# AntreasAntoniou/HowToTrainYourMAMLPytorch

Measured on AMD Instinct MI355X. Metric: meta-tasks/sec, higher is better.
Workload: dtype bf16; 1 GPU; model=maml++_miniimagenet_5w1s, global_batch=128, tasks_per_gpu=128, ways=5, shots=1, targets=15, filters=48, inner_steps=5, msl=True, parallelism=task-dp1

## Files before the change

### howtotrainyourmamlpytorch_amd/ops/hip/bindings.cpp

```cpp
#include <torch/extension.h>
#include <vector>

std::vector<torch::Tensor> bn_act_fwd(torch::Tensor x, torch::Tensor gamma,
                                      torch::Tensor beta, double eps,
                                      double slope, bool act);
std::vector<torch::Tensor> bn_act_bwd(torch::Tensor dy, torch::Tensor x,
                                      torch::Tensor mean, torch::Tensor rstd,
                                      torch::Tensor gamma, torch::Tensor beta,
                                      double slope, bool act);
std::vector<torch::Tensor> bn_act_pool_fwd(torch::Tensor x, torch::Tensor gamma,
                                           torch::Tensor beta, double eps,
                                           double slope,
                                           c10::optional<torch::Tensor> sums_in);
std::vector<torch::Tensor> bn_act_pool_bwd(torch::Tensor dyp, torch::Tensor mask,
                                           torch::Tensor x, torch::Tensor mean,
                                           torch::Tensor rstd, torch::Tensor gamma,
                                           torch::Tensor beta, double slope);
std::vector<torch::Tensor> maxpool2x2_fwd(torch::Tensor x);
torch::Tensor maxpool2x2_bwd(torch::Tensor dy, torch::Tensor mask, long H, long W);
std::vector<torch::Tensor> ce_fwd(torch::Tensor logits, torch::Tensor labels);
torch::Tensor ce_bwd(torch::Tensor probs, torch::Tensor labels, torch::Tensor gtask);
std::vector<torch::Tensor> ce_dbwd(torch::Tensor probs, torch::Tensor labels,
                                   torch::Tensor gdl, torch::Tensor gtask);
std::vector<torch::Tensor> bn_act_dbwd(torch::Tensor x, torch::Tensor u,
                                       torch::Tensor gx, torch::Tensor mean,
                                       torch::Tensor rstd, torch::Tensor gamma,
                                       torch::Tensor beta, torch::Tensor ggam,
                                       torch::Tensor gbet, double slope, bool act);
std::vector<torch::Tensor> ln_act_fwd(torch::Tensor x, torch::Tensor bias,
                                      double eps, double slope, bool act);
std::vector<torch::Tensor> ln_act_bwd(torch::Tensor dy, torch::Tensor x,
                                      torch::Tensor mean, torch::Tensor rstd,
                                      torch::Tensor bias, double slope, bool act);
std::vector<torch::Tensor> ln_act_dbwd(torch::Tensor x, torch::Tensor dy,
                                       torch::Tensor gx, torch::Tensor gb,
                                       torch::Tensor mean, torch::Tensor rstd,
                                       torch::Tensor bias, double slope, bool act);
torch::Tensor lslr_fwd(torch::Tensor arena, torch::Tensor grad, torch::Tensor lr_vec);
std::vector<torch::Tensor> lslr_bwd(torch::Tensor gout, torch::Tensor grad,
                                    torch::Tensor lr_vec);
torch::Tensor tconv_repack(torch::Tensor w, bool dgrad);
std::vector<torch::Tensor> tconv_mm(torch::Tensor x, torch::Tensor wp,
                                    c10::optional<torch::Tensor> bias, long pad,
// ... 37 lines not shown
torch::Tensor gavgpool_bwd(torch::Tensor dy, long H, long W);
void adam_step(std::vector<torch::Tensor> params,
               std::vector<torch::Tensor> grads,
               std::vector<torch::Tensor> exp_avgs,
               std::vector<torch::Tensor> exp_avg_sqs,
               long step, double lr, double beta1, double beta2, double eps,
               double weight_decay, double clamp_v);

PYBIND11_MODULE(TORCH_EXTENSION_NAME, m) {
  m.def("bn_act_fwd", &bn_act_fwd, "fused task-batched BN+leakyReLU fwd");
  m.def("bn_act_bwd", &bn_act_bwd, "fused task-batched BN+leakyReLU bwd");
  m.def("bn_act_pool_fwd", &bn_act_pool_fwd, "fused BN+leakyReLU+maxpool fwd");
  m.def("bn_act_pool_bwd", &bn_act_pool_bwd, "fused BN+leakyReLU+maxpool bwd");
  m.def("maxpool2x2_fwd", &maxpool2x2_fwd, "NHWC maxpool 2x2 fwd");
  m.def("maxpool2x2_bwd", &maxpool2x2_bwd, "NHWC maxpool 2x2 bwd");
  m.def("ce_fwd", &ce_fwd, "fused softmax-CE fwd");
  m.def("ce_dbwd", &ce_dbwd, "softmax-CE double-backward");
  m.def("bn_act_dbwd", &bn_act_dbwd, "BN+leakyReLU analytic double-backward");
  m.def("ce_bwd", &ce_bwd, "fused softmax-CE bwd");
  m.def("ln_act_fwd", &ln_act_fwd, "fused task-batched LayerNorm+bias+leakyReLU fwd");
  m.def("ln_act_bwd", &ln_act_bwd, "fused task-batched LayerNorm+bias+leakyReLU bwd");
  m.def("ln_act_dbwd", &ln_act_dbwd, "LayerNorm+bias+leakyReLU analytic double-backward");
  m.def("lslr_fwd", &lslr_fwd, "fused LSLR arena update fwd");
  m.def("lslr_bwd", &lslr_bwd, "fused LSLR arena update bwd");
  m.def("tconv_repack", &tconv_repack, "repack conv weights for MFMA (fwd/dgrad)");
  m.def("tconv_mm", &tconv_mm, "task-batched MFMA 3x3 conv fwd/dgrad");
  m.def("tconv_wgrad", &tconv_wgrad, "task-batched MFMA 3x3 conv wgrad");
  m.def("tconv_repack_v2", &tconv_repack_v2,
        "repack conv weights into the v2 swizzled LDS image");
  m.def("tconv_mm_v2", &tconv_mm_v2,
        "async-pipelined MFMA 3x3 conv fwd/dgrad (v2)");
  m.def("tconv_wgrad_v2", &tconv_wgrad_v2,
        "async-pipelined wgrad via k-contiguous operand transposes (v2)");
// ... 24 lines not shown
```

### howtotrainyourmamlpytorch_amd/ops/hip/bn_act.hip

```cpp

#include "common.h"

using namespace maml355;

template <typename scalar_t>
__global__ void bn_sums_vec_kernel(const scalar_t* __restrict__ x,
                                   float* __restrict__ partials,
                                   int T, long M, int C, int rows_per_block) {
  const int c8n = C / 8;
  const int rows_in_block = blockDim.x / c8n;
  const int c8 = threadIdx.x % c8n;
  const int rg = threadIdx.x / c8n;
  const int t = blockIdx.x;
  const long row0 = (long)blockIdx.y * rows_per_block;
  extern __shared__ float ls[];
  float s[8] = {0}, q[8] = {0};
  if (rg < rows_in_block) {
    const scalar_t* xt = x + (long)t * M * C + c8 * 8;
    const long row_end = min(row0 + rows_per_block, M);
    for (long m = row0 + rg; m < row_end; m += rows_in_block) {
      float v[8];
      load8(xt + m * C, v);
#pragma unroll
      for (int j = 0; j < 8; ++j) { s[j] += v[j]; q[j] += v[j] * v[j]; }
// ... 17 lines not shown
      }
    }
    __syncthreads();
    n_ = step;
  }
  if (rg == 0) {
    float* pt = partials + (((long)t * gridDim.y + blockIdx.y) * 2) * C;
#pragma unroll
    for (int j = 0; j < 8; ++j) {
      pt[c8 * 8 + j] = ls[0 * C + c8 * 8 + j];
      pt[C + c8 * 8 + j] = ls[1 * C + c8 * 8 + j];
    }
  }
}

__global__ void bn_reduce2_kernel(const float* __restrict__ partials,
                                  float* __restrict__ sums, int T, int nblk,
                                  int C) {
  const int i = blockIdx.x * blockDim.x + threadIdx.x;
  if (i >= T * C) return;
  const int t = i / C, c = i % C;
  float s = 0.f, q = 0.f;
  for (int b = 0; b < nblk; ++b) {
    const float* p = partials + (((long)t * nblk + b) * 2) * C;
    s += p[c];
    q += p[C + c];
  }
  sums[((long)t * 2 + 0) * C + c] = s;
  sums[((long)t * 2 + 1) * C + c] = q;
}

template <typename scalar_t, bool PER_TASK_AFFINE, bool ACT>
__global__ void bn_norm_act_vec_kernel(const scalar_t* __restrict__ x,
                                       scalar_t* __restrict__ y,
                                       const float* __restrict__ mean,
                                       const float* __restrict__ rstd,
                                       const float* __restrict__ gamma,
                                       const float* __restrict__ beta,
                                       int T, long M, int C, float slope,
                                       int rows_per_block) {
  const int c8n = C / 8;
  const int rows_in_block = blockDim.x / c8n;
  const int c8 = threadIdx.x % c8n;
  const int rg = threadIdx.x / c8n;
// ... 515 lines not shown
    }
    const float s1 = bsums[((long)t * 2 + 0) * C + c];
    const float s2 = bsums[((long)t * 2 + 1) * C + c];
    dx[i] = from_f32<scalar_t>(g * rs * (d - s1 * invM - xh * s2 * invM));
  }
}

#include <torch/extension.h>
#include <ATen/cuda/CUDAContext.h>

namespace {

constexpr int kRowsPerBlock = 256;
constexpr int kThreads = 256;

template <typename scalar_t>
void bn_fwd_impl(const torch::Tensor& x, const torch::Tensor& gamma,
                 const torch::Tensor& beta, torch::Tensor& y,
                 torch::Tensor& sums, torch::Tensor& mean, torch::Tensor& var,
                 torch::Tensor& rstd, double eps, double slope, bool act,
                 int T, long M, int C) {
  auto stream = at::cuda::getCurrentCUDAStream();
  const bool per_task = gamma.dim() == 2;
  const bool vec = (C % 8 == 0) && C <= 512;
  const int cpad = ((C + WAVE - 1) / WAVE) * WAVE;
  dim3 sums_grid(T, (unsigned)((M + kRowsPerBlock - 1) / kRowsPerBlock));
  const int threads = cpad * std::max<int>(1, kThreads / cpad);
  const int lds_bytes = 2 * threads * sizeof(float);
  if (vec) {
    const int rpb = 1024;
    const int nb = (int)((M + rpb - 1) / rpb);
    dim3 g(T, (unsigned)nb);
    auto partials = torch::empty({T, nb, 2, C},
                                 x.options().dtype(torch::kFloat32));
    hipLaunchKernelGGL((bn_sums_vec_kernel<scalar_t>), g, dim3(256),
                       16384, stream.stream(),
                       reinterpret_cast<const scalar_t*>(x.data_ptr()),
                       partials.data_ptr<float>(), T, M, C, rpb);
    hipLaunchKernelGGL(bn_reduce2_kernel, dim3((T * C + 255) / 256), dim3(256),
                       0, stream.stream(), partials.data_ptr<float>(),
                       sums.data_ptr<float>(), T, nb, C);
  } else
  hipLaunchKernelGGL((bn_sums_kernel<scalar_t>), sums_grid, dim3(threads),
                     lds_bytes, stream.stream(),
                     reinterpret_cast<const scalar_t*>(x.data_ptr()), sums.data_ptr<float>(), T, M, C,
                     kRowsPerBlock);
  const int fin_threads = 256;
  const int fin_blocks = (T * C + fin_threads - 1) / fin_threads;
  hipLaunchKernelGGL(bn_finalize_kernel, dim3(fin_blocks), dim3(fin_threads), 0,
                     stream.stream(), sums.data_ptr<float>(),
                     mean.data_ptr<float>(), var.data_ptr<float>(),
                     rstd.data_ptr<float>(), T, M, C, (float)eps);
  const long total = (long)T * M * C;
#define LAUNCH_NORM(PT, ACT_)                                                  \
  do {                                                                         \
    if (vec) {                                                                 \
// ... 12 lines not shown
                         reinterpret_cast<scalar_t*>(y.data_ptr()),            \
                         mean.data_ptr<float>(), rstd.data_ptr<float>(),       \
                         gamma.data_ptr<float>(), beta.data_ptr<float>(),      \
                         T, M, C, (float)slope);                               \
    }                                                                          \
  } while (0)
  if (per_task) { if (act) LAUNCH_NORM(true, true); else LAUNCH_NORM(true, false); }
  else { if (act) LAUNCH_NORM(false, true); else LAUNCH_NORM(false, false); }
#undef LAUNCH_NORM
}

template <typename scalar_t>
void bn_bwd_impl(const torch::Tensor& dy, const torch::Tensor& x,
                 const torch::Tensor& mean, const torch::Tensor& rstd,
                 const torch::Tensor& gamma, const torch::Tensor& beta,
                 torch::Tensor& bsums, torch::Tensor& dx, double slope,
                 bool act, int T, long M, int C) {
  auto stream = at::cuda::getCurrentCUDAStream();
  const bool per_task = gamma.dim() == 2;
  const bool vec = (C % 8 == 0) && C <= 512;
  const int cpad = ((C + WAVE - 1) / WAVE) * WAVE;
  dim3 sums_grid(T, (unsigned)((M + kRowsPerBlock - 1) / kRowsPerBlock));
  const int threads = cpad * std::max<int>(1, kThreads / cpad);
  const int lds_bytes = 2 * threads * sizeof(float);
  const long total = (long)T * M * C;
#define LAUNCH_BWD(PT, ACT_)                                                   \
  do {                                                                         \
    if (vec) {                                                                 \
      const int nb = (int)((M + 1023) / 1024);                                 \
      dim3 gs(T, (unsigned)nb);                                                \
      auto partials = torch::empty({T, nb, 2, C},                              \
                                   x.options().dtype(torch::kFloat32));        \
      hipLaunchKernelGGL((bn_bwd_sums_vec_kernel<scalar_t, PT, ACT_>),         \
                         gs, dim3(256), 16384,                                 \
                         stream.stream(),                                      \
                         reinterpret_cast<const scalar_t*>(dy.data_ptr()),     \
                         reinterpret_cast<const scalar_t*>(x.data_ptr()),      \
                         mean.data_ptr<float>(), rstd.data_ptr<float>(),       \
                         gamma.data_ptr<float>(), beta.data_ptr<float>(),      \
                         partials.data_ptr<float>(), T, M, C, (float)slope,    \
                         1024);                                                \
      hipLaunchKernelGGL(bn_reduce2_kernel, dim3((T * C + 255) / 256),         \
                         dim3(256), 0, stream.stream(),                        \
                         partials.data_ptr<float>(),                           \
                         bsums.data_ptr<float>(), T, nb, C);                   \
      hipLaunchKernelGGL((bn_bwd_dx_vec_kernel<scalar_t, PT, ACT_>),           \
                         sums_grid, dim3(256), 0, stream.stream(),             \
                         reinterpret_cast<const scalar_t*>(dy.data_ptr()),     \
                         reinterpret_cast<const scalar_t*>(x.data_ptr()),      \
                         reinterpret_cast<scalar_t*>(dx.data_ptr()),           \
                         mean.data_ptr<float>(), rstd.data_ptr<float>(),       \
                         gamma.data_ptr<float>(), beta.data_ptr<float>(),      \
                         bsums.data_ptr<float>(), T, M, C, (float)slope,       \
                         kRowsPerBlock);                                       \
      break;                                                                   \
    }                                                                          \
    hipLaunchKernelGGL((bn_bwd_sums_kernel<scalar_t, PT, ACT_>), sums_grid,    \
                       dim3(threads), lds_bytes, stream.stream(),              \
                       reinterpret_cast<const scalar_t*>(dy.data_ptr()),       \
                       reinterpret_cast<const scalar_t*>(x.data_ptr()),        \
// ... 14 lines not shown
  if (per_task) { if (act) LAUNCH_BWD(true, true); else LAUNCH_BWD(true, false); }
  else { if (act) LAUNCH_BWD(false, true); else LAUNCH_BWD(false, false); }
#undef LAUNCH_BWD
}

}

std::vector<torch::Tensor> bn_act_fwd(torch::Tensor x, torch::Tensor gamma,
                                      torch::Tensor beta, double eps,
                                      double slope, bool act) {
  TORCH_CHECK(x.is_cuda() && x.dim() == 3 && x.is_contiguous());
  const int T = (int)x.size(0);
  const long M = x.size(1);
  const int C = (int)x.size(2);
  auto opts = x.options().dtype(torch::kFloat32);
  auto sums = torch::zeros({T, 2, C}, opts);
  auto mean = torch::empty({T, C}, opts);
  auto var = torch::empty({T, C}, opts);
  auto rstd = torch::empty({T, C}, opts);
  auto y = torch::empty_like(x);
  auto gc = gamma.contiguous().to(torch::kFloat32);
  auto bc = beta.contiguous().to(torch::kFloat32);
  if (x.scalar_type() == torch::kFloat32) {
    bn_fwd_impl<float>(x, gc, bc, y, sums, mean, var, rstd, eps, slope, act, T, M, C);
  } else if (x.scalar_type() == torch::kBFloat16) {
    bn_fwd_impl<__hip_bfloat16>(x, gc, bc, y, sums, mean, var, rstd, eps, slope, act, T, M, C);
  } else {
    TORCH_CHECK(false, "bn_act_fwd: unsupported dtype");
  }
  return {y, mean, var, rstd};
}

std::vector<torch::Tensor> bn_act_bwd(torch::Tensor dy, torch::Tensor x,
                                      torch::Tensor mean, torch::Tensor rstd,
                                      torch::Tensor gamma, torch::Tensor beta,
                                      double slope, bool act) {
  TORCH_CHECK(dy.is_cuda() && dy.dim() == 3);
  auto dyc = dy.contiguous();
  const int T = (int)x.size(0);
  const long M = x.size(1);
  const int C = (int)x.size(2);
  auto opts = x.options().dtype(torch::kFloat32);
  auto bsums = torch::zeros({T, 2, C}, opts);
  auto dx = torch::empty_like(x);
  auto gc = gamma.contiguous().to(torch::kFloat32);
  auto bc = beta.contiguous().to(torch::kFloat32);
  if (x.scalar_type() == torch::kFloat32) {
    bn_bwd_impl<float>(dyc, x, mean, rstd, gc, bc, bsums, dx, slope, act, T, M, C);
  } else if (x.scalar_type() == torch::kBFloat16) {
    bn_bwd_impl<__hip_bfloat16>(dyc, x, mean, rstd, gc, bc, bsums, dx, slope, act, T, M, C);
  } else {
    TORCH_CHECK(false, "bn_act_bwd: unsupported dtype");
  }
  return {dx, bsums.select(1, 1).clone(), bsums.select(1, 0).clone()};
}

std::vector<torch::Tensor> bn_act_pool_fwd(torch::Tensor x, torch::Tensor gamma,
                                           torch::Tensor beta, double eps,
                                           double slope,
                                           c10::optional<torch::Tensor> sums_in) {
  TORCH_CHECK(x.is_cuda() && x.dim() == 5 && x.is_contiguous());
  const int T = (int)x.size(0), NB = (int)x.size(1), H = (int)x.size(2),
            W = (int)x.size(3), C = (int)x.size(4);
  TORCH_CHECK(C % 8 == 0 && C <= 512, "bn_act_pool_fwd needs C % 8 == 0");
  const long M = (long)NB * H * W;
  const int Ho = H / 2, Wo = W / 2;
  auto fopts = x.options().dtype(torch::kFloat32);
  const bool have_sums = sums_in.has_value() && sums_in->numel() == T * 2 * C;
  auto sums = have_sums ? sums_in->contiguous()
                        : torch::zeros({T, 2, C}, fopts);
  auto mean = torch::empty({T, C}, fopts);
  auto var = torch::empty({T, C}, fopts);
  auto rstd = torch::empty({T, C}, fopts);
  auto y = torch::empty({T, NB, Ho, Wo, C}, x.options());
  auto mask = torch::empty({T, NB, Ho, Wo, C}, x.options().dtype(torch::kUInt8));
  auto gc = gamma.contiguous().to(torch::kFloat32);
  auto bc = beta.contiguous().to(torch::kFloat32);
  const bool per_task = gamma.dim() == 2;
  auto stream = at::cuda::getCurrentCUDAStream();
  const int rpb = 1024;
  dim3 gsums(T, (unsigned)((M + rpb - 1) / rpb));
  const long ptotal = (long)T * NB * Ho * Wo * (C / 8);
  const int pblocks = (int)std::min<long>((ptotal + 255) / 256, 4096);

#define LAUNCH_BNP(ST, PT)                                                     \
  do {                                                                         \
    if (!have_sums) {                                                          \
      const int nb_ = (int)((M + rpb - 1) / rpb);                              \
      auto partials = torch::empty({T, nb_, 2, C}, fopts);                     \
      hipLaunchKernelGGL((bn_sums_vec_kernel<ST>), gsums, dim3(256),           \
                         16384, stream.stream(),                               \
                         reinterpret_cast<const ST*>(x.data_ptr()),            \
                         partials.data_ptr<float>(), T, M, C, rpb);            \
      hipLaunchKernelGGL(bn_reduce2_kernel, dim3((T * C + 255) / 256),         \
                         dim3(256), 0, stream.stream(),                        \
                         partials.data_ptr<float>(),                           \
                         sums.data_ptr<float>(), T, nb_, C);                   \
    }                                                                          \
    const int fin_blocks = (T * C + 255) / 256;                                \
    hipLaunchKernelGGL(bn_finalize_kernel, dim3(fin_blocks), dim3(256), 0,     \
                       stream.stream(), sums.data_ptr<float>(),                \
                       mean.data_ptr<float>(), var.data_ptr<float>(),          \
                       rstd.data_ptr<float>(), T, M, C, (float)eps);           \
    hipLaunchKernelGGL((bn_norm_act_pool_vec_kernel<ST, PT>), dim3(pblocks),   \
                       dim3(256), 0, stream.stream(),                          \
                       reinterpret_cast<const ST*>(x.data_ptr()),              \
                       reinterpret_cast<ST*>(y.data_ptr()),                    \
                       mask.data_ptr<unsigned char>(),                         \
                       mean.data_ptr<float>(), rstd.data_ptr<float>(),         \
                       gc.data_ptr<float>(), bc.data_ptr<float>(),             \
                       T, NB, H, W, C, Ho, Wo, (float)slope);                  \
  } while (0)
// ... 8 lines not shown
  }
#undef LAUNCH_BNP
  return {y, mask, mean, var, rstd};
}

std::vector<torch::Tensor> bn_act_pool_bwd(torch::Tensor dyp, torch::Tensor mask,
                                           torch::Tensor x, torch::Tensor mean,
                                           torch::Tensor rstd, torch::Tensor gamma,
                                           torch::Tensor beta, double slope) {
  TORCH_CHECK(x.is_cuda() && x.dim() == 5 && x.is_contiguous());
  const int T = (int)x.size(0), NB = (int)x.size(1), H = (int)x.size(2),
            W = (int)x.size(3), C = (int)x.size(4);
  TORCH_CHECK(C % 8 == 0 && C <= 512);
  const long M = (long)NB * H * W;
  auto fopts = x.options().dtype(torch::kFloat32);
  auto bsums = torch::zeros({T, 2, C}, fopts);
  auto dx = torch::empty_like(x);
  auto gc = gamma.contiguous().to(torch::kFloat32);
  auto bc = beta.contiguous().to(torch::kFloat32);
  auto dypc = dyp.contiguous();
  const bool per_task = gamma.dim() == 2;
  auto stream = at::cuda::getCurrentCUDAStream();
  const int rpb = 1024;
  dim3 g(T, (unsigned)((M + rpb - 1) / rpb));

#define LAUNCH_BPB(ST, PT)                                                     \
  do {                                                                         \
    const int nb_ = (int)((M + rpb - 1) / rpb);                                \
    auto partials = torch::empty({T, nb_, 2, C}, fopts);                       \
    hipLaunchKernelGGL((bn_pool_bwd_sums_vec_kernel<ST, PT>), g, dim3(256),    \
                       16384, stream.stream(),                                 \
                       reinterpret_cast<const ST*>(dypc.data_ptr()),           \
                       mask.data_ptr<unsigned char>(),                         \
                       reinterpret_cast<const ST*>(x.data_ptr()),              \
                       mean.data_ptr<float>(), rstd.data_ptr<float>(),         \
                       gc.data_ptr<float>(), bc.data_ptr<float>(),             \
                       partials.data_ptr<float>(), T, NB, H, W, C,             \
                       (float)slope, rpb);                                     \
    hipLaunchKernelGGL(bn_reduce2_kernel, dim3((T * C + 255) / 256),           \
                       dim3(256), 0, stream.stream(),                          \
                       partials.data_ptr<float>(),                             \
                       bsums.data_ptr<float>(), T, nb_, C);                    \
    hipLaunchKernelGGL((bn_pool_bwd_dx_vec_kernel<ST, PT>), g, dim3(256), 0,   \
                       stream.stream(),                                        \
                       reinterpret_cast<const ST*>(dypc.data_ptr()),           \
                       mask.data_ptr<unsigned char>(),                         \
                       reinterpret_cast<const ST*>(x.data_ptr()),              \
                       reinterpret_cast<ST*>(dx.data_ptr()),                   \
                       mean.data_ptr<float>(), rstd.data_ptr<float>(),         \
                       gc.data_ptr<float>(), bc.data_ptr<float>(),             \
                       bsums.data_ptr<float>(), T, NB, H, W, C, (float)slope,  \
                       rpb);                                                   \
  } while (0)

  if (x.scalar_type() == torch::kFloat32) {
    if (per_task) LAUNCH_BPB(float, true); else LAUNCH_BPB(float, false);
  } else if (x.scalar_type() == torch::kBFloat16) {
    if (per_task) LAUNCH_BPB(__hip_bfloat16, true);
    else LAUNCH_BPB(__hip_bfloat16, false);
  } else {
    TORCH_CHECK(false, "bn_act_pool_bwd: unsupported dtype");
  }
#undef LAUNCH_BPB
  return {dx, bsums.select(1, 1).clone(), bsums.select(1, 0).clone()};
}
```

### howtotrainyourmamlpytorch_amd/ops/hip/bn_dbwd.hip

```cpp

#include "common.h"
#include <torch/extension.h>
#include <ATen/cuda/CUDAContext.h>

using namespace maml355;
using bf16 = __hip_bfloat16;

template <typename scalar_t, bool PER_TASK_AFFINE>
__global__ void bn_dbwd_sums_kernel(const scalar_t* __restrict__ x,
                                    const scalar_t* __restrict__ u,
                                    const scalar_t* __restrict__ gx,
                                    const float* __restrict__ mean,
                                    const float* __restrict__ rstd,
                                    const float* __restrict__ gamma,
                                    const float* __restrict__ beta,
                                    float* __restrict__ partials,
                                    int T, long M, int C, float slope,
                                    bool act, int rows_per_block) {
  const int cpad = ((C + WAVE - 1) / WAVE) * WAVE;
  const int rows_in_block = blockDim.x / cpad;
  const int c = threadIdx.x % cpad;
  const int rgroup = threadIdx.x / cpad;
  const int t = blockIdx.x;
  const long row0 = (long)blockIdx.y * rows_per_block;
// ... 31 lines not shown
      s1 += lds[0 * n + rr * cpad + c];
      s2 += lds[1 * n + rr * cpad + c];
      G += lds[2 * n + rr * cpad + c];
      Gxh += lds[3 * n + rr * cpad + c];
      Gu += lds[4 * n + rr * cpad + c];
    }
    float* pt = partials + (((long)t * gridDim.y + blockIdx.y) * 5) * C;
    pt[0 * C + c] = s1;
    pt[1 * C + c] = s2;
    pt[2 * C + c] = G;
    pt[3 * C + c] = Gxh;
    pt[4 * C + c] = Gu;
  }
}

__global__ void bn_reduce5_kernel(const float* __restrict__ partials,
                                  float* __restrict__ sums, int T, int nblk,
                                  int C) {
  const int i = blockIdx.x * blockDim.x + threadIdx.x;
  if (i >= T * C) return;
  const int t = i / C, c = i % C;
  float acc[5] = {0.f, 0.f, 0.f, 0.f, 0.f};
  for (int b = 0; b < nblk; ++b) {
    const float* p = partials + (((long)t * nblk + b) * 5) * C;
#pragma unroll
    for (int k = 0; k < 5; ++k) acc[k] += p[k * C + c];
  }
#pragma unroll
  for (int k = 0; k < 5; ++k) sums[((long)t * 5 + k) * C + c] = acc[k];
}

template <typename scalar_t, bool PER_TASK_AFFINE>
__global__ void bn_dbwd_apply_kernel(const scalar_t* __restrict__ x,
                                     const scalar_t* __restrict__ u,
                                     const scalar_t* __restrict__ gx,
                                     scalar_t* __restrict__ d_u,
                                     scalar_t* __restrict__ d_x,
                                     const float* __restrict__ mean,
                                     const float* __restrict__ rstd,
                                     const float* __restrict__ gamma,
                                     const float* __restrict__ beta,
                                     const float* __restrict__ ggam,
                                     const float* __restrict__ gbet,
                                     const float* __restrict__ sums,
// ... 28 lines not shown
    const float du = mask * (g * r * gcent + gg * xh + gb);
    const float dxv = g * r * r *
                          (-xh * (Gu - s1 * G - s2 * Gxh) - s2 * gcent -
                           ucent * Gxh) +
                      gg * r * ucent;
    d_u[i] = from_f32<scalar_t>(du);
    d_x[i] = from_f32<scalar_t>(dxv);
  }
}

namespace {
constexpr int kRowsPerBlockD = 256;
constexpr int kThreadsD = 256;
}

std::vector<torch::Tensor> bn_act_dbwd(torch::Tensor x, torch::Tensor u,
                                       torch::Tensor gx, torch::Tensor mean,
                                       torch::Tensor rstd, torch::Tensor gamma,
                                       torch::Tensor beta, torch::Tensor ggam,
                                       torch::Tensor gbet, double slope,
                                       bool act) {
  TORCH_CHECK(x.is_cuda() && x.dim() == 3 && x.is_contiguous());
  const int T = (int)x.size(0);
  const long M = x.size(1);
  const int C = (int)x.size(2);
  auto fopts = x.options().dtype(torch::kFloat32);
  auto sums = torch::zeros({T, 5, C}, fopts);
  auto d_u = torch::empty_like(x);
  auto d_x = torch::empty_like(x);
  auto gc = gamma.contiguous().to(torch::kFloat32);
  auto bc = beta.contiguous().to(torch::kFloat32);
  auto ggc = ggam.contiguous().to(torch::kFloat32);
  auto gbc = gbet.contiguous().to(torch::kFloat32);
  auto uc = u.contiguous();
  auto gxc = gx.contiguous();
  const bool per_task = gamma.dim() == 2;
  auto stream = at::cuda::getCurrentCUDAStream();
  const int cpad = ((C + WAVE - 1) / WAVE) * WAVE;
  const int threads = cpad * std::max<int>(1, kThreadsD / cpad);
  dim3 sums_grid(T, (unsigned)((M + kRowsPerBlockD - 1) / kRowsPerBlockD));
  const int lds_bytes = 5 * threads * (int)sizeof(float);
  const long total = (long)T * M * C;

#define LAUNCH_DB(ST, PT)                                                      \
  do {                                                                         \
    const int nblk = (int)sums_grid.y;                                         \
    auto partials = torch::empty({T, nblk, 5, C}, fopts);                      \
    hipLaunchKernelGGL((bn_dbwd_sums_kernel<ST, PT>), sums_grid,               \
                       dim3(threads), lds_bytes, stream.stream(),              \
                       reinterpret_cast<const ST*>(x.data_ptr()),              \
                       reinterpret_cast<const ST*>(uc.data_ptr()),             \
                       reinterpret_cast<const ST*>(gxc.data_ptr()),            \
                       mean.data_ptr<float>(), rstd.data_ptr<float>(),         \
                       gc.data_ptr<float>(), bc.data_ptr<float>(),             \
                       partials.data_ptr<float>(), T, M, C, (float)slope, act, \
                       kRowsPerBlockD);                                        \
    hipLaunchKernelGGL(bn_reduce5_kernel, dim3((T * C + 255) / 256),           \
                       dim3(256), 0, stream.stream(),                          \
                       partials.data_ptr<float>(), sums.data_ptr<float>(),     \
                       T, nblk, C);                                            \
    hipLaunchKernelGGL((bn_dbwd_apply_kernel<ST, PT>),                         \
                       dim3(ew_grid(total, kThreadsD)), dim3(kThreadsD), 0,    \
                       stream.stream(),                                        \
                       reinterpret_cast<const ST*>(x.data_ptr()),              \
                       reinterpret_cast<const ST*>(uc.data_ptr()),             \
                       reinterpret_cast<const ST*>(gxc.data_ptr()),            \
                       reinterpret_cast<ST*>(d_u.data_ptr()),                  \
                       reinterpret_cast<ST*>(d_x.data_ptr()),                  \
                       mean.data_ptr<float>(), rstd.data_ptr<float>(),         \
                       gc.data_ptr<float>(), bc.data_ptr<float>(),             \
                       ggc.data_ptr<float>(), gbc.data_ptr<float>(),           \
                       sums.data_ptr<float>(), T, M, C, (float)slope, act);    \
  } while (0)

  if (x.scalar_type() == torch::kFloat32) {
    if (per_task) LAUNCH_DB(float, true); else LAUNCH_DB(float, false);
  } else if (x.scalar_type() == torch::kBFloat16) {
    if (per_task) LAUNCH_DB(bf16, true); else LAUNCH_DB(bf16, false);
  } else {
    TORCH_CHECK(false, "bn_act_dbwd: unsupported dtype");
  }
#undef LAUNCH_DB
  return {d_u, d_x, sums};
}
```

### howtotrainyourmamlpytorch_amd/ops/hip/pool.hip

```cpp

#include "common.h"
#include <torch/extension.h>
#include <ATen/cuda/CUDAContext.h>

using namespace maml355;

template <typename scalar_t>
__global__ void maxpool_fwd_kernel(const scalar_t* __restrict__ x,
                                   scalar_t* __restrict__ y,
                                   unsigned char* __restrict__ mask,
                                   long N, int H, int W, int C, int Ho, int Wo) {
  const long total = N * (long)Ho * Wo * C;
  for (long i = (long)blockIdx.x * blockDim.x + threadIdx.x; i < total;
       i += grid_stride()) {
    const int c = (int)(i % C);
    long r = i / C;
    const int wo = (int)(r % Wo); r /= Wo;
    const int ho = (int)(r % Ho); r /= Ho;
    const long n = r;
    const long base = ((n * H + 2 * ho) * W + 2 * wo) * C + c;
    float best = to_f32(x[base]);
    int arg = 0;
    const float v01 = to_f32(x[base + C]);
    if (v01 > best) { best = v01; arg = 1; }
// ... 95 lines not shown
      float dv[8], out[8];
      load8(&dy[o], dv);
#pragma unroll
      for (int j = 0; j < 8; ++j) {
        const int mj = (int)((mpack >> (8 * j)) & 0xff);
        out[j] = (mj == arg) ? dv[j] : 0.f;
      }
      store8(&dx[ibase], out);
    } else {
      float z[8] = {0, 0, 0, 0, 0, 0, 0, 0};
      store8(&dx[ibase], z);
    }
  }
}

std::vector<torch::Tensor> maxpool2x2_fwd(torch::Tensor x) {
  TORCH_CHECK(x.is_cuda() && x.dim() == 4 && x.is_contiguous());
  const long N = x.size(0);
  const int H = (int)x.size(1), W = (int)x.size(2), C = (int)x.size(3);
  const int Ho = H / 2, Wo = W / 2;
  auto y = torch::empty({N, Ho, Wo, C}, x.options());
  auto mask = torch::empty({N, Ho, Wo, C}, x.options().dtype(torch::kUInt8));
  const bool vec = (C % 8 == 0);
  const long total = N * (long)Ho * Wo * (vec ? C / 8 : C);
  auto stream = at::cuda::getCurrentCUDAStream();
#define LAUNCH_PF(st)                                                          \
  do {                                                                         \
    if (vec)                                                                   \
      hipLaunchKernelGGL((maxpool_fwd_vec_kernel<st>),                         \
                         dim3(ew_grid(total, 256)), dim3(256), 0,              \
// ... 55 lines not shown
```

### howtotrainyourmamlpytorch_amd/ops/hip_autograd.py

```python

from __future__ import annotations

import collections
import os

import torch

from . import hip_ext
from . import reference as ref


def _ext():
    e = hip_ext()
    assert e is not None, "hip_autograd used without loaded extension"
    return e


class _BNBwdFn(torch.autograd.Function):

    @staticmethod
    def forward(ctx, x3, gamma, beta, u, mean, rstd, slope, act):
        dx, dgamma_t, dbeta_t = _ext().bn_act_bwd(
            u, x3, mean, rstd, gamma.float(), beta.float(), slope, act)
        ctx.save_for_backward(x3, gamma, beta, u, mean, rstd)
        ctx.slope, ctx.act = slope, act
        return dx, dgamma_t, dbeta_t

    @staticmethod
    def backward(ctx, gx, ggam_t, gbet_t):
        x3, gamma, beta, u, mean, rstd = ctx.saved_tensors
        T, M, C = x3.shape
        if ggam_t is None:
            ggam_t = torch.zeros(T, C, device=x3.device, dtype=torch.float32)
        if gbet_t is None:
            gbet_t = torch.zeros(T, C, device=x3.device, dtype=torch.float32)
        d_u, d_x, sums = _ext().bn_act_dbwd(
            x3, u, gx.contiguous(), mean, rstd, gamma.float(), beta.float(),
            ggam_t, gbet_t, ctx.slope, ctx.act)
        s = sums / M
        d_gamma_t = rstd * M * (s[:, 4] - s[:, 0] * s[:, 2] - s[:, 1] * s[:, 3])
        per_task = gamma.dim() == 2
        d_gamma = d_gamma_t if per_task else d_gamma_t.sum(0)
        return (d_x, d_gamma.to(gamma.dtype), None, d_u, None, None, None, None)


class _BNActFn(torch.autograd.Function):

    @staticmethod
    def forward(ctx, x3, gamma, beta, eps, slope, act):
        y, mean, var, rstd = _ext().bn_act_fwd(x3, gamma.float(), beta.float(),
                                               eps, slope, act)
        ctx.save_for_backward(x3, mean, rstd, gamma, beta)
        ctx.eps, ctx.slope, ctx.act = eps, slope, act
        ctx.mark_non_differentiable(mean, var)
        return y, mean, var
# ... 105 lines not shown
                         "[T, H, W, C], got %s" % (tuple(bias.shape),))
    return _LNActFn.apply(x.contiguous(), b2.float().contiguous(), eps,
                          negative_slope, apply_act)


class _PoolBwdFn(torch.autograd.Function):
    @staticmethod
    def forward(ctx, dy, mask, H, W):
        ctx.save_for_backward(mask)
        ctx.HW = (H, W)
        return _ext().maxpool2x2_bwd(dy, mask, H, W)

    @staticmethod
    def backward(ctx, ddx):
        (mask,) = ctx.saved_tensors
        g = _gather_by_mask(ddx.contiguous(), mask)
        return g, None, None, None


def _gather_by_mask(x4, mask):
    N, H, W, C = x4.shape
    Ho, Wo = mask.shape[1], mask.shape[2]
    win = x4[:, :2 * Ho, :2 * Wo, :].reshape(N, Ho, 2, Wo, 2, C)
    win = win.permute(0, 1, 3, 5, 2, 4).reshape(N, Ho, Wo, C, 4)
    return torch.gather(win, 4, mask.long().unsqueeze(-1)).squeeze(-1)


class _PoolFn(torch.autograd.Function):
    @staticmethod
    def forward(ctx, x4):
        y, mask = _ext().maxpool2x2_fwd(x4)
# ... 414 lines not shown
```

Before: 698.0 tasks/s.

## Fuse BN double-backward glue and pool-gather into HIP kernels, drop zero-inits

Moves the d_gamma computation of BN double-backward into the reduce kernel and adds a vectorized dbwd sums kernel. It also replaces the PyTorch permute/gather maxpool double-backward with a dedicated NHWC gather kernel. BN backward now writes dgamma/dbeta directly from the reduce kernel instead of cloning slices, replaces zero-initialised sum buffers with empty ones, and unrolls the reduce loops so partial loads are issued ahead of the adds. The aim is fewer small launches, allocations and Python-side elementwise ops in the second-order MAML graph, at the cost of more custom kernel code behind an env flag.

Result: faster. 726.9 tasks/s (median of 6 runs) (+4.1%).

```diff
diff --git a/howtotrainyourmamlpytorch_amd/ops/hip/bindings.cpp b/howtotrainyourmamlpytorch_amd/ops/hip/bindings.cpp
--- a/howtotrainyourmamlpytorch_amd/ops/hip/bindings.cpp
+++ b/howtotrainyourmamlpytorch_amd/ops/hip/bindings.cpp
@@ -18,6 +18,7 @@
                                            torch::Tensor beta, double slope);
 std::vector<torch::Tensor> maxpool2x2_fwd(torch::Tensor x);
 torch::Tensor maxpool2x2_bwd(torch::Tensor dy, torch::Tensor mask, long H, long W);
+torch::Tensor maxpool2x2_gather(torch::Tensor x, torch::Tensor mask);
 std::vector<torch::Tensor> ce_fwd(torch::Tensor logits, torch::Tensor labels);
 torch::Tensor ce_bwd(torch::Tensor probs, torch::Tensor labels, torch::Tensor gtask);
 std::vector<torch::Tensor> ce_dbwd(torch::Tensor probs, torch::Tensor labels,
@@ -27,6 +28,11 @@
                                        torch::Tensor rstd, torch::Tensor gamma,
                                        torch::Tensor beta, torch::Tensor ggam,
                                        torch::Tensor gbet, double slope, bool act);
+std::vector<torch::Tensor> bn_act_dbwd_full(
+    torch::Tensor x, torch::Tensor u, torch::Tensor gx, torch::Tensor mean,
+    torch::Tensor rstd, torch::Tensor gamma, torch::Tensor beta,
+    c10::optional<torch::Tensor> ggam, c10::optional<torch::Tensor> gbet,
+    double slope, bool act);
 std::vector<torch::Tensor> ln_act_fwd(torch::Tensor x, torch::Tensor bias,
                                       double eps, double slope, bool act);
 std::vector<torch::Tensor> ln_act_bwd(torch::Tensor dy, torch::Tensor x,
@@ -94,9 +100,13 @@
   m.def("bn_act_pool_bwd", &bn_act_pool_bwd, "fused BN+leakyReLU+maxpool bwd");
   m.def("maxpool2x2_fwd", &maxpool2x2_fwd, "NHWC maxpool 2x2 fwd");
   m.def("maxpool2x2_bwd", &maxpool2x2_bwd, "NHWC maxpool 2x2 bwd");
+  m.def("maxpool2x2_gather", &maxpool2x2_gather,
+        "NHWC 2x2 window gather through a saved argmax mask");
   m.def("ce_fwd", &ce_fwd, "fused softmax-CE fwd");
   m.def("ce_dbwd", &ce_dbwd, "softmax-CE double-backward");
   m.def("bn_act_dbwd", &bn_act_dbwd, "BN+leakyReLU analytic double-backward");
+  m.def("bn_act_dbwd_full", &bn_act_dbwd_full,
+        "BN+leakyReLU double-backward with d_gamma_t, optional ggam/gbet");
   m.def("ce_bwd", &ce_bwd, "fused softmax-CE bwd");
   m.def("ln_act_fwd", &ln_act_fwd, "fused task-batched LayerNorm+bias+leakyReLU fwd");
   m.def("ln_act_bwd", &ln_act_bwd, "fused task-batched LayerNorm+bias+leakyReLU bwd");
diff --git a/howtotrainyourmamlpytorch_amd/ops/hip/bn_act.hip b/howtotrainyourmamlpytorch_amd/ops/hip/bn_act.hip
--- a/howtotrainyourmamlpytorch_amd/ops/hip/bn_act.hip
+++ b/howtotrainyourmamlpytorch_amd/ops/hip/bn_act.hip
@@ -55,20 +55,37 @@
   }
 }
 
+constexpr int kAhead2 = 16;
 __global__ void bn_reduce2_kernel(const float* __restrict__ partials,
                                   float* __restrict__ sums, int T, int nblk,
-                                  int C) {
+                                  int C, float* __restrict__ out0,
+                                  float* __restrict__ out1) {
   const int i = blockIdx.x * blockDim.x + threadIdx.x;
   if (i >= T * C) return;
   const int t = i / C, c = i % C;
   float s = 0.f, q = 0.f;
-  for (int b = 0; b < nblk; ++b) {
-    const float* p = partials + (((long)t * nblk + b) * 2) * C;
-    s += p[c];
-    q += p[C + c];
+  for (int b0 = 0; b0 < nblk; b0 += kAhead2) {
+    float vs[kAhead2], vq[kAhead2];
+#pragma unroll
+    for (int a = 0; a < kAhead2; ++a) {
+      if (b0 + a < nblk) {
+        const float* p = partials + (((long)t * nblk + b0 + a) * 2) * C;
+        vs[a] = p[c];
+        vq[a] = p[C + c];
+      }
+    }
+#pragma unroll
+    for (int a = 0; a < kAhead2; ++a) {
+      if (b0 + a < nblk) {
+        s += vs[a];
+        q += vq[a];
+      }
+    }
   }
   sums[((long)t * 2 + 0) * C + c] = s;
   sums[((long)t * 2 + 1) * C + c] = q;
+  if (out0 != nullptr) out0[i] = s;
+  if (out1 != nullptr) out1[i] = q;
 }
 
 template <typename scalar_t, bool PER_TASK_AFFINE, bool ACT>
@@ -614,6 +631,8 @@
 constexpr int kRowsPerBlock = 256;
 constexpr int kThreads = 256;
 
+inline bool bn_vec_ok(int C) { return (C % 8 == 0) && C <= 512; }
+
 template <typename scalar_t>
 void bn_fwd_impl(const torch::Tensor& x, const torch::Tensor& gamma,
                  const torch::Tensor& beta, torch::Tensor& y,
@@ -622,7 +641,7 @@
                  int T, long M, int C) {
   auto stream = at::cuda::getCurrentCUDAStream();
   const bool per_task = gamma.dim() == 2;
-  const bool vec = (C % 8 == 0) && C <= 512;
+  const bool vec = bn_vec_ok(C);
   const int cpad = ((C + WAVE - 1) / WAVE) * WAVE;
   dim3 sums_grid(T, (unsigned)((M + kRowsPerBlock - 1) / kRowsPerBlock));
   const int threads = cpad * std::max<int>(1, kThreads / cpad);
@@ -639,7 +658,8 @@
                        partials.data_ptr<float>(), T, M, C, rpb);
     hipLaunchKernelGGL(bn_reduce2_kernel, dim3((T * C + 255) / 256), dim3(256),
                        0, stream.stream(), partials.data_ptr<float>(),
-                       sums.data_ptr<float>(), T, nb, C);
+                       sums.data_ptr<float>(), T, nb, C, (float*)nullptr,
+                       (float*)nullptr);
   } else
   hipLaunchKernelGGL((bn_sums_kernel<scalar_t>), sums_grid, dim3(threads),
                      lds_bytes, stream.stream(),
@@ -682,11 +702,12 @@
 void bn_bwd_impl(const torch::Tensor& dy, const torch::Tensor& x,
                  const torch::Tensor& mean, const torch::Tensor& rstd,
                  const torch::Tensor& gamma, const torch::Tensor& beta,
-                 torch::Tensor& bsums, torch::Tensor& dx, double slope,
+                 torch::Tensor& bsums, torch::Tensor& dx,
+                 torch::Tensor& dgamma_t, torch::Tensor& dbeta_t, double slope,
                  bool act, int T, long M, int C) {
   auto stream = at::cuda::getCurrentCUDAStream();
   const bool per_task = gamma.dim() == 2;
-  const bool vec = (C % 8 == 0) && C <= 512;
+  const bool vec = bn_vec_ok(C);
   const int cpad = ((C + WAVE - 1) / WAVE) * WAVE;
   dim3 sums_grid(T, (unsigned)((M + kRowsPerBlock - 1) / kRowsPerBlock));
   const int threads = cpad * std::max<int>(1, kThreads / cpad);
@@ -711,7 +732,9 @@
       hipLaunchKernelGGL(bn_reduce2_kernel, dim3((T * C + 255) / 256),         \
                          dim3(256), 0, stream.stream(),                        \
                          partials.data_ptr<float>(),                           \
-                         bsums.data_ptr<float>(), T, nb, C);                   \
+                         bsums.data_ptr<float>(), T, nb, C,                    \
+                         dbeta_t.data_ptr<float>(),                            \
+                         dgamma_t.data_ptr<float>());                          \
       hipLaunchKernelGGL((bn_bwd_dx_vec_kernel<scalar_t, PT, ACT_>),           \
                          sums_grid, dim3(256), 0, stream.stream(),             \
                          reinterpret_cast<const scalar_t*>(dy.data_ptr()),     \
@@ -756,7 +779,8 @@
   const long M = x.size(1);
   const int C = (int)x.size(2);
   auto opts = x.options().dtype(torch::kFloat32);
-  auto sums = torch::zeros({T, 2, C}, opts);
+  auto sums = bn_vec_ok(C) ? torch::empty({T, 2, C}, opts)
+                           : torch::zeros({T, 2, C}, opts);
   auto mean = torch::empty({T, C}, opts);
   auto var = torch::empty({T, C}, opts);
   auto rstd = torch::empty({T, C}, opts);
@@ -783,17 +807,27 @@
   const long M = x.size(1);
   const int C = (int)x.size(2);
   auto opts = x.options().dtype(torch::kFloat32);
-  auto bsums = torch::zeros({T, 2, C}, opts);
+  const bool vec = bn_vec_ok(C);
+  auto bsums = vec ? torch::empty({T, 2, C}, opts)
+                   : torch::zeros({T, 2, C}, opts);
+  torch::Tensor dgamma_t, dbeta_t;
+  if (vec) {
+    dgamma_t = torch::empty({T, C}, opts);
+    dbeta_t = torch::empty({T, C}, opts);
+  }
   auto dx = torch::empty_like(x);
   auto gc = gamma.contiguous().to(torch::kFloat32);
   auto bc = beta.contiguous().to(torch::kFloat32);
   if (x.scalar_type() == torch::kFloat32) {
-    bn_bwd_impl<float>(dyc, x, mean, rstd, gc, bc, bsums, dx, slope, act, T, M, C);
+    bn_bwd_impl<float>(dyc, x, mean, rstd, gc, bc, bsums, dx, dgamma_t,
+                       dbeta_t, slope, act, T, M, C);
   } else if (x.scalar_type() == torch::kBFloat16) {
-    bn_bwd_impl<__hip_bfloat16>(dyc, x, mean, rstd, gc, bc, bsums, dx, slope, act, T, M, C);
+    bn_bwd_impl<__hip_bfloat16>(dyc, x, mean, rstd, gc, bc, bsums, dx,
+                                dgamma_t, dbeta_t, slope, act, T, M, C);
   } else {
     TORCH_CHECK(false, "bn_act_bwd: unsupported dtype");
   }
+  if (vec) return {dx, dgamma_t, dbeta_t};
   return {dx, bsums.select(1, 1).clone(), bsums.select(1, 0).clone()};
 }
 
@@ -810,7 +844,7 @@
   auto fopts = x.options().dtype(torch::kFloat32);
   const bool have_sums = sums_in.has_value() && sums_in->numel() == T * 2 * C;
   auto sums = have_sums ? sums_in->contiguous()
-                        : torch::zeros({T, 2, C}, fopts);
+                        : torch::empty({T, 2, C}, fopts);
   auto mean = torch::empty({T, C}, fopts);
   auto var = torch::empty({T, C}, fopts);
   auto rstd = torch::empty({T, C}, fopts);
@@ -837,7 +871,8 @@
       hipLaunchKernelGGL(bn_reduce2_kernel, dim3((T * C + 255) / 256),         \
                          dim3(256), 0, stream.stream(),                        \
                          partials.data_ptr<float>(),                           \
-                         sums.data_ptr<float>(), T, nb_, C);                   \
+                         sums.data_ptr<float>(), T, nb_, C, (float*)nullptr,   \
+                         (float*)nullptr);                                     \
     }                                                                          \
     const int fin_blocks = (T * C + 255) / 256;                                \
     hipLaunchKernelGGL(bn_finalize_kernel, dim3(fin_blocks), dim3(256), 0,     \
@@ -876,7 +911,9 @@
   TORCH_CHECK(C % 8 == 0 && C <= 512);
   const long M = (long)NB * H * W;
   auto fopts = x.options().dtype(torch::kFloat32);
-  auto bsums = torch::zeros({T, 2, C}, fopts);
+  auto bsums = torch::empty({T, 2, C}, fopts);
+  auto dgamma_t = torch::empty({T, C}, fopts);
+  auto dbeta_t = torch::empty({T, C}, fopts);
   auto dx = torch::empty_like(x);
   auto gc = gamma.contiguous().to(torch::kFloat32);
   auto bc = beta.contiguous().to(torch::kFloat32);
@@ -902,7 +939,9 @@
     hipLaunchKernelGGL(bn_reduce2_kernel, dim3((T * C + 255) / 256),           \
                        dim3(256), 0, stream.stream(),                          \
                        partials.data_ptr<float>(),                             \
-                       bsums.data_ptr<float>(), T, nb_, C);                    \
+                       bsums.data_ptr<float>(), T, nb_, C,                     \
+                       dbeta_t.data_ptr<float>(),                              \
+                       dgamma_t.data_ptr<float>());                            \
     hipLaunchKernelGGL((bn_pool_bwd_dx_vec_kernel<ST, PT>), g, dim3(256), 0,   \
                        stream.stream(),                                        \
                        reinterpret_cast<const ST*>(dypc.data_ptr()),           \
@@ -924,5 +963,5 @@
     TORCH_CHECK(false, "bn_act_pool_bwd: unsupported dtype");
   }
 #undef LAUNCH_BPB
-  return {dx, bsums.select(1, 1).clone(), bsums.select(1, 0).clone()};
-}
+  return {dx, dgamma_t, dbeta_t};
+}
diff --git a/howtotrainyourmamlpytorch_amd/ops/hip/bn_dbwd.hip b/howtotrainyourmamlpytorch_amd/ops/hip/bn_dbwd.hip
--- a/howtotrainyourmamlpytorch_amd/ops/hip/bn_dbwd.hip
+++ b/howtotrainyourmamlpytorch_amd/ops/hip/bn_dbwd.hip
@@ -69,20 +69,46 @@
   }
 }
 
-__global__ void bn_reduce5_kernel(const float* __restrict__ partials,
-                                  float* __restrict__ sums, int T, int nblk,
-                                  int C) {
+constexpr int kAhead5 = 8;
+__global__ void __launch_bounds__(256)
+bn_reduce5_kernel(const float* __restrict__ partials, float* __restrict__ sums,
+                  int T, int nblk, int C, const float* __restrict__ rstd,
+                  float* __restrict__ dgamma_t, float Mf, float invM) {
   const int i = blockIdx.x * blockDim.x + threadIdx.x;
   if (i >= T * C) return;
   const int t = i / C, c = i % C;
   float acc[5] = {0.f, 0.f, 0.f, 0.f, 0.f};
-  for (int b = 0; b < nblk; ++b) {
-    const float* p = partials + (((long)t * nblk + b) * 5) * C;
-#pragma unroll
-    for (int k = 0; k < 5; ++k) acc[k] += p[k * C + c];
+  for (int b0 = 0; b0 < nblk; b0 += kAhead5) {
+    float v[kAhead5][5];
+#pragma unroll
+    for (int a = 0; a < kAhead5; ++a) {
+      if (b0 + a < nblk) {
+        const float* p = partials + (((long)t * nblk + b0 + a) * 5) * C;
+#pragma unroll
+        for (int k = 0; k < 5; ++k) v[a][k] = p[k * C + c];
+      }
+    }
+#pragma unroll
+    for (int a = 0; a < kAhead5; ++a) {
+      if (b0 + a < nblk) {
+#pragma unroll
+        for (int k = 0; k < 5; ++k) acc[k] += v[a][k];
+      }
+    }
   }
 #pragma unroll
   for (int k = 0; k < 5; ++k) sums[((long)t * 5 + k) * C + c] = acc[k];
+  if (dgamma_t != nullptr) {
+#pragma clang fp contract(off)
+    const float s0 = acc[0] * invM, s1 = acc[1] * invM, s2 = acc[2] * invM,
+                s3 = acc[3] * invM, s4 = acc[4] * invM;
+    const float rm = rstd[i] * Mf;
+    const float p02 = s0 * s2;
+    const float d1 = s4 - p02;
+    const float p13 = s1 * s3;
+    const float d2 = d1 - p13;
+    dgamma_t[i] = rm * d2;
+  }
 }
 
 template <typename scalar_t, bool PER_TASK_AFFINE>
@@ -141,18 +167,103 @@
 constexpr int kThreadsD = 256;
 }
 
-std::vector<torch::Tensor> bn_act_dbwd(torch::Tensor x, torch::Tensor u,
-                                       torch::Tensor gx, torch::Tensor mean,
-                                       torch::Tensor rstd, torch::Tensor gamma,
-                                       torch::Tensor beta, torch::Tensor ggam,
-                                       torch::Tensor gbet, double slope,
-                                       bool act) {
+template <typename scalar_t, bool PER_TASK_AFFINE>
+__global__ void bn_dbwd_sums_vec_kernel(
+    const scalar_t* __restrict__ x, const scalar_t* __restrict__ u,
+    const scalar_t* __restrict__ gx, const float* __restrict__ mean,
+    const float* __restrict__ rstd, const float* __restrict__ gamma,
+    const float* __restrict__ beta,
+    float* __restrict__ partials,
+    long M, int C, float slope, bool act, int R, int slices_per_block,
+    int nslice) {
+  const int c8n = C / 8;
+  const int c8 = threadIdx.x % c8n;
+  const int chain = threadIdx.x / c8n;
+  const int sl = chain / R, rg = chain % R;
+  const int t = blockIdx.x;
+  const int slice = blockIdx.y * slices_per_block + sl;
+  const bool live = sl < slices_per_block && slice < nslice;
+  const int c0 = c8 * 8;
+  extern __shared__ float ls[];
+  if (live) {
+    float mu[8], r[8], g[8], b[8];
+#pragma unroll
+    for (int j = 0; j < 8; ++j) {
+      const long tc = (long)t * C + c0 + j;
+      mu[j] = mean[tc]; r[j] = rstd[tc];
+      g[j] = PER_TASK_AFFINE ? gamma[tc] : gamma[c0 + j];
+      b[j] = PER_TASK_AFFINE ? beta[tc] : beta[c0 + j];
+    }
+    float s1[8] = {0}, s2[8] = {0}, G[8] = {0}, Gxh[8] = {0}, Gu[8] = {0};
+    const long base = (long)t * M * C + c0;
+    const long row0 = (long)slice * kRowsPerBlockD;
+    const long row_end = min(row0 + kRowsPerBlockD, M);
+    for (long m = row0 + rg; m < row_end; m += R) {
+      float xv[8], uv[8], gxv[8];
+      load8(x + base + m * C, xv);
+      load8(u + base + m * C, uv);
+      load8(gx + base + m * C, gxv);
+#pragma unroll
+      for (int j = 0; j < 8; ++j) {
+#pragma clang fp contract(off)
+        const float xh = (xv[j] - mu[j]) * r[j];
+        float up = uv[j];
+        if (act) up = up * ((__builtin_fmaf(g[j], xh, b[j]) > 0.f) ? 1.f : slope);
+        const float gv = gxv[j];
+        const float upxh = up * xh;
+        s1[j] = s1[j] + up;
+        s2[j] = s2[j] + upxh;
+        G[j] = G[j] + gv;
+        Gxh[j] = __builtin_fmaf(gv, xh, Gxh[j]);
+        Gu[j] = __builtin_fmaf(gv, up, Gu[j]);
+      }
+    }
+    float* lc = ls + (long)chain * 5 * C + c0;
+#pragma unroll
+    for (int j = 0; j < 8; ++j) {
+      lc[0 * C + j] = s1[j];
+      lc[1 * C + j] = s2[j];
+      lc[2 * C + j] = G[j];
+      lc[3 * C + j] = Gxh[j];
+      lc[4 * C + j] = Gu[j];
+    }
+  }
+  __syncthreads();
+  if (live && rg == 0) {
+    float* pt = partials + (((long)t * nslice + slice) * 5) * C + c0;
+#pragma unroll
+    for (int k = 0; k < 5; ++k) {
+#pragma unroll
+      for (int j = 0; j < 8; ++j) {
+        float v = ls[((long)chain * 5 + k) * C + c0 + j];
+        for (int rr = 1; rr < R; ++rr)
+          v += ls[((long)(chain + rr) * 5 + k) * C + c0 + j];
+        pt[k * C + j] = v;
+      }
+    }
+  }
+}
+
+namespace {
+
+std::vector<torch::Tensor> dbwd_run(const torch::Tensor& x,
+                                    const torch::Tensor& u,
+                                    const torch::Tensor& gx,
+                                    const torch::Tensor& mean,
+                                    const torch::Tensor& rstd,
+                                    const torch::Tensor& gamma,
+                                    const torch::Tensor& beta,
+                                    const torch::Tensor& ggam,
+                                    const torch::Tensor& gbet, double slope,
+                                    bool act, bool vec_sums,
+                                    torch::Tensor d_gamma_t) {
   TORCH_CHECK(x.is_cuda() && x.dim() == 3 && x.is_contiguous());
   const int T = (int)x.size(0);
   const long M = x.size(1);
   const int C = (int)x.size(2);
+  TORCH_CHECK(u.numel() == x.numel() && gx.numel() == x.numel());
   auto fopts = x.options().dtype(torch::kFloat32);
-  auto sums = torch::zeros({T, 5, C}, fopts);
+  auto sums = torch::empty({T, 5, C}, fopts);
   auto d_u = torch::empty_like(x);
   auto d_x = torch::empty_like(x);
   auto gc = gamma.contiguous().to(torch::kFloat32);
@@ -168,11 +279,34 @@
   dim3 sums_grid(T, (unsigned)((M + kRowsPerBlockD - 1) / kRowsPerBlockD));
   const int lds_bytes = 5 * threads * (int)sizeof(float);
   const long total = (long)T * M * C;
+  const int R = threads / cpad;
+  const int c8n = std::max(1, C / 8);
+  const int spb = std::max(1, std::min(kThreadsD / c8n / R, 16));
+  const int vblocks = ((int)sums_grid.y + spb - 1) / spb;
+  const int vlds_bytes = spb * R * 5 * C * (int)sizeof(float);
+  const bool vec = vec_sums && (C % 8 == 0) && C <= 512 && vblocks <= 65535;
+  TORCH_CHECK(!vec || spb * R * c8n <= kThreadsD);
+  const float Mf = (float)M;
+  const float invM = 1.0f / Mf;
+  const float* rstd_p = d_gamma_t.defined() ? rstd.data_ptr<float>() : nullptr;
+  float* dgam_p = d_gamma_t.defined() ? d_gamma_t.data_ptr<float>() : nullptr;
 
 #define LAUNCH_DB(ST, PT)                                                      \
   do {                                                                         \
     const int nblk = (int)sums_grid.y;                                         \
     auto partials = torch::empty({T, nblk, 5, C}, fopts);                      \
+    if (vec)                                                                   \
+      hipLaunchKernelGGL((bn_dbwd_sums_vec_kernel<ST, PT>),                    \
+                         dim3(T, vblocks), dim3(kThreadsD), vlds_bytes,        \
+                         stream.stream(),                                      \
+                         reinterpret_cast<const ST*>(x.data_ptr()),            \
+                         reinterpret_cast<const ST*>(uc.data_ptr()),           \
+                         reinterpret_cast<const ST*>(gxc.data_ptr()),          \
+                         mean.data_ptr<float>(), rstd.data_ptr<float>(),       \
+                         gc.data_ptr<float>(), bc.data_ptr<float>(),           \
+                         partials.data_ptr<float>(), M, C, (float)slope, act,  \
+                         R, spb, nblk);                                        \
+    else                                                                       \
     hipLaunchKernelGGL((bn_dbwd_sums_kernel<ST, PT>), sums_grid,               \
                        dim3(threads), lds_bytes, stream.stream(),              \
                        reinterpret_cast<const ST*>(x.data_ptr()),              \
@@ -185,7 +319,7 @@
     hipLaunchKernelGGL(bn_reduce5_kernel, dim3((T * C + 255) / 256),           \
                        dim3(256), 0, stream.stream(),                          \
                        partials.data_ptr<float>(), sums.data_ptr<float>(),     \
-                       T, nblk, C);                                            \
+                       T, nblk, C, rstd_p, dgam_p, Mf, invM);                  \
     hipLaunchKernelGGL((bn_dbwd_apply_kernel<ST, PT>),                         \
                        dim3(ew_grid(total, kThreadsD)), dim3(kThreadsD), 0,    \
                        stream.stream(),                                        \
@@ -210,3 +344,37 @@
 #undef LAUNCH_DB
   return {d_u, d_x, sums};
 }
+
+}
+
+std::vector<torch::Tensor> bn_act_dbwd(torch::Tensor x, torch::Tensor u,
+                                       torch::Tensor gx, torch::Tensor mean,
+                                       torch::Tensor rstd, torch::Tensor gamma,
+                                       torch::Tensor beta, torch::Tensor ggam,
+                                       torch::Tensor gbet, double slope,
+                                       bool act) {
+  return dbwd_run(x, u, gx, mean, rstd, gamma, beta, ggam, gbet, slope, act,
+                  false, torch::Tensor());
+}
+
+std::vector<torch::Tensor> bn_act_dbwd_full(
+    torch::Tensor x, torch::Tensor u, torch::Tensor gx, torch::Tensor mean,
+    torch::Tensor rstd, torch::Tensor gamma, torch::Tensor beta,
+    c10::optional<torch::Tensor> ggam, c10::optional<torch::Tensor> gbet,
+    double slope, bool act) {
+  TORCH_CHECK(x.is_cuda() && x.dim() == 3);
+  const long T = x.size(0), C = x.size(2);
+  TORCH_CHECK(mean.numel() == T * C && rstd.numel() == T * C);
+  auto fopts = x.options().dtype(torch::kFloat32);
+  const bool has_gg = ggam.has_value() && ggam->defined();
+  const bool has_gb = gbet.has_value() && gbet->defined();
+  TORCH_CHECK((!has_gg || ggam->numel() == T * C) &&
+              (!has_gb || gbet->numel() == T * C));
+  torch::Tensor zero;
+  if (!has_gg || !has_gb) zero = torch::zeros({T, C}, fopts);
+  auto d_gamma_t = torch::empty({T, C}, fopts);
+  auto out = dbwd_run(x, u, gx, mean, rstd, gamma, beta,
+                      has_gg ? *ggam : zero, has_gb ? *gbet : zero, slope, act,
+                      true, d_gamma_t);
+  return {out[0], out[1], d_gamma_t, out[2]};
+}
diff --git a/howtotrainyourmamlpytorch_amd/ops/hip/pool.hip b/howtotrainyourmamlpytorch_amd/ops/hip/pool.hip
--- a/howtotrainyourmamlpytorch_amd/ops/hip/pool.hip
+++ b/howtotrainyourmamlpytorch_amd/ops/hip/pool.hip
@@ -133,6 +133,66 @@
   }
 }
 
+template <typename scalar_t>
+__global__ void maxpool_gather_vec_kernel(const scalar_t* __restrict__ x,
+                                          const unsigned char* __restrict__ mask,
+                                          scalar_t* __restrict__ y,
+                                          unsigned total, int H, int W, int C,
+                                          int Ho, int Wo) {
+  const unsigned c8n = C / 8;
+  for (unsigned i = blockIdx.x * blockDim.x + threadIdx.x; i < total;
+       i += blockDim.x * gridDim.x) {
+    const unsigned c8 = i % c8n;
+    unsigned r = i / c8n;
+    const unsigned wo = r % Wo; r /= Wo;
+    const unsigned ho = r % Ho;
+    const unsigned n = r / Ho;
+    const long base = (((long)n * H + 2 * ho) * W + 2 * wo) * C + c8 * 8;
+    float v[4][8], out[8];
+    load8(&x[base], v[0]);
+    load8(&x[base + C], v[1]);
+    load8(&x[base + (long)W * C], v[2]);
+    load8(&x[base + (long)W * C + C], v[3]);
+    const long o = (long)i * 8;
+    const unsigned long long mp = *(const unsigned long long*)&mask[o];
+#pragma unroll
+    for (int j = 0; j < 8; ++j) {
+      const int a = (int)((mp >> (8 * j)) & 3);
+      out[j] = a == 0 ? v[0][j] : a == 1 ? v[1][j] : a == 2 ? v[2][j] : v[3][j];
+    }
+    store8(&y[o], out);
+  }
+}
+
+torch::Tensor maxpool2x2_gather(torch::Tensor x, torch::Tensor mask) {
+  TORCH_CHECK(x.is_cuda() && x.dim() == 4 && mask.dim() == 4);
+  auto xc = x.contiguous();
+  auto mc = mask.contiguous();
+  const long N = x.size(0);
+  const int H = (int)x.size(1), W = (int)x.size(2), C = (int)x.size(3);
+  const int Ho = H / 2, Wo = W / 2;
+  TORCH_CHECK(mask.size(0) == N && mask.size(1) == Ho && mask.size(2) == Wo &&
+              mask.size(3) == C && mask.scalar_type() == torch::kUInt8);
+  auto y = torch::empty({N, Ho, Wo, C}, x.options());
+  TORCH_CHECK(C % 8 == 0, "maxpool2x2_gather needs C % 8 == 0");
+  const long total = N * (long)Ho * Wo * (C / 8);
+  TORCH_CHECK(total < (1L << 31), "maxpool2x2_gather: too many positions");
+  if (total == 0) return y;
+  auto stream = at::cuda::getCurrentCUDAStream();
+#define LAUNCH_PG(st)                                                          \
+  hipLaunchKernelGGL((maxpool_gather_vec_kernel<st>),                          \
+                     dim3(ew_grid(total, 256)), dim3(256), 0, stream.stream(), \
+                     reinterpret_cast<const st*>(xc.data_ptr()),               \
+                     mc.data_ptr<unsigned char>(),                             \
+                     reinterpret_cast<st*>(y.data_ptr()), (unsigned)total, H,  \
+                     W, C, Ho, Wo)
+  if (x.scalar_type() == torch::kFloat32) LAUNCH_PG(float);
+  else if (x.scalar_type() == torch::kBFloat16) LAUNCH_PG(__hip_bfloat16);
+  else TORCH_CHECK(false, "maxpool2x2_gather: unsupported dtype");
+#undef LAUNCH_PG
+  return y;
+}
+
 std::vector<torch::Tensor> maxpool2x2_fwd(torch::Tensor x) {
   TORCH_CHECK(x.is_cuda() && x.dim() == 4 && x.is_contiguous());
   const long N = x.size(0);
diff --git a/howtotrainyourmamlpytorch_amd/ops/hip_autograd.py b/howtotrainyourmamlpytorch_amd/ops/hip_autograd.py
--- a/howtotrainyourmamlpytorch_amd/ops/hip_autograd.py
+++ b/howtotrainyourmamlpytorch_amd/ops/hip_autograd.py
@@ -14,6 +14,10 @@
     e = hip_ext()
     assert e is not None, "hip_autograd used without loaded extension"
     return e
+
+
+def _dbwd_glue_off() -> bool:
+    return os.environ.get("MAML355_BNPOOL_DBWD", "1") != "0"
 
 
 class _BNBwdFn(torch.autograd.Function):
@@ -24,21 +28,29 @@
             u, x3, mean, rstd, gamma.float(), beta.float(), slope, act)
         ctx.save_for_backward(x3, gamma, beta, u, mean, rstd)
         ctx.slope, ctx.act = slope, act
+        ctx.set_materialize_grads(False)
         return dx, dgamma_t, dbeta_t
 
     @staticmethod
     def backward(ctx, gx, ggam_t, gbet_t):
         x3, gamma, beta, u, mean, rstd = ctx.saved_tensors
         T, M, C = x3.shape
-        if ggam_t is None:
-            ggam_t = torch.zeros(T, C, device=x3.device, dtype=torch.float32)
-        if gbet_t is None:
-            gbet_t = torch.zeros(T, C, device=x3.device, dtype=torch.float32)
-        d_u, d_x, sums = _ext().bn_act_dbwd(
-            x3, u, gx.contiguous(), mean, rstd, gamma.float(), beta.float(),
-            ggam_t, gbet_t, ctx.slope, ctx.act)
-        s = sums / M
-        d_gamma_t = rstd * M * (s[:, 4] - s[:, 0] * s[:, 2] - s[:, 1] * s[:, 3])
+        if gx is None:
+            gx = torch.zeros_like(x3)
+        if _dbwd_glue_off():
+            d_u, d_x, d_gamma_t, _ = _ext().bn_act_dbwd_full(
+                x3, u, gx.contiguous(), mean, rstd, gamma.float(),
+                beta.float(), ggam_t, gbet_t, ctx.slope, ctx.act)
+        else:
+            if ggam_t is None:
+                ggam_t = torch.zeros(T, C, device=x3.device, dtype=torch.float32)
+            if gbet_t is None:
+                gbet_t = torch.zeros(T, C, device=x3.device, dtype=torch.float32)
+            d_u, d_x, sums = _ext().bn_act_dbwd(
+                x3, u, gx.contiguous(), mean, rstd, gamma.float(), beta.float(),
+                ggam_t, gbet_t, ctx.slope, ctx.act)
+            s = sums / M
+            d_gamma_t = rstd * M * (s[:, 4] - s[:, 0] * s[:, 2] - s[:, 1] * s[:, 3])
         per_task = gamma.dim() == 2
         d_gamma = d_gamma_t if per_task else d_gamma_t.sum(0)
         return (d_x, d_gamma.to(gamma.dtype), None, d_u, None, None, None, None)
@@ -174,7 +186,10 @@
     @staticmethod
     def backward(ctx, ddx):
         (mask,) = ctx.saved_tensors
-        g = _gather_by_mask(ddx.contiguous(), mask)
+        if mask.shape[-1] % 8 == 0 and _dbwd_glue_off():
+            g = _ext().maxpool2x2_gather(ddx.contiguous(), mask)
+        else:
+            g = _gather_by_mask(ddx.contiguous(), mask)
         return g, None, None, None
 
 
```
